# hpcaitech/CachedEmbedding

Measured on AMD Instinct MI355X. Metric: embedding lookups/sec (cache op + EmbeddingBag fwd + bwd/SGD), Criteo-1TB table @1% cache, higher is better.
Workload: dtype f32

## Files before the change

### cachedembedding_amd/csrc/ce_bag.hip

```cpp
#include <stdlib.h>

#include <algorithm>

#include "ce_common.h"

namespace ce {

#ifdef CE_ABLATIONS
#define CE_DBG(x) (x)
#else
#define CE_DBG(x) 0
#endif

struct BagParams {
  const float* weight;
  float* dst;
  const float* grad_out;
  const int64_t* indices;
  const void* offsets;
  const float* psw;
  int64_t nnz;
  int32_t num_bags;
  int32_t rowlen;
  int32_t g_log2;
// ... 303 lines not shown
  return lo;
}

template <typename KT> struct KeyOps;
template <> struct KeyOps<uint32_t> {
  static __device__ __forceinline__ uint32_t make(uint32_t row, int i) { return (row << 10) | (uint32_t)i; }
  static __device__ __forceinline__ uint32_t row(uint32_t k) { return k >> 10; }
  static __device__ __forceinline__ int idx(uint32_t k) { return (int)(k & 1023u); }
  static __device__ __forceinline__ uint32_t invalid() { return 0xffffffffu; }
  static __device__ __forceinline__ uint32_t row_invalid() { return 0x3fffffu; }
};
template <> struct KeyOps<unsigned long long> {
  static __device__ __forceinline__ unsigned long long make(uint32_t row, int i) {
    return ((unsigned long long)row << 32) | (uint32_t)i;
  }
  static __device__ __forceinline__ uint32_t row(unsigned long long k) { return (uint32_t)(k >> 32); }
  static __device__ __forceinline__ int idx(unsigned long long k) { return (int)(uint32_t)k; }
  static __device__ __forceinline__ unsigned long long invalid() { return ~0ull; }
  static __device__ __forceinline__ uint32_t row_invalid() { return 0xffffffffu; }
};

template <typename KT>
__device__ __forceinline__ KT shfl_xor_key(KT v, int m) { return __shfl_xor(v, m); }
template <>
__device__ __forceinline__ unsigned long long shfl_xor_key<unsigned long long>(unsigned long long v, int m) {
  const unsigned lo = __shfl_xor((unsigned)v, m), hi = __shfl_xor((unsigned)(v >> 32), m);
  return ((unsigned long long)hi << 32) | lo;
}

template <typename KT>
__device__ __forceinline__ void tile_sort_1024(KT (&key)[4], KT* lds, int tid) {
  for (int k = 2; k <= kBwdTile; k <<= 1) {
    for (int j = k >> 1; j > 0; j >>= 1) {
      if (j >= 256) {
#pragma unroll
        for (int r = 0; r < 4; ++r) lds[tid * 4 + r] = key[r];
        __syncthreads();
#pragma unroll
        for (int r = 0; r < 4; ++r) {
          const int i = tid * 4 + r;
          const KT other = lds[i ^ j];
          const bool lower = (i & j) == 0, up = (i & k) == 0;
          const KT lo = key[r] < other ? key[r] : other, hi = key[r] < other ? other : key[r];
          key[r] = (lower == up) ? lo : hi;
        }
        __syncthreads();
      } else if (j >= 4) {
#pragma unroll
        for (int r = 0; r < 4; ++r) {
          const int i = tid * 4 + r;
          const KT other = shfl_xor_key<KT>(key[r], j >> 2);
          const bool lower = (i & j) == 0, up = (i & k) == 0;
          const KT lo = key[r] < other ? key[r] : other, hi = key[r] < other ? other : key[r];
          key[r] = (lower == up) ? lo : hi;
        }
      } else {
#pragma unroll
        for (int r = 0; r < 4; ++r) {
          if (r & j) continue;
          const bool up = ((tid * 4 + r) & k) == 0;
          const KT a = key[r], b = key[r | j];
          if ((a > b) == up) {
            key[r] = b;
            key[r | j] = a;
          }
        }
      }
    }
  }
#pragma unroll
  for (int r = 0; r < 4; ++r) lds[tid * 4 + r] = key[r];
  __syncthreads();
}

constexpr int kSegLen = 16384;
constexpr int kSegKeys = 16;
#ifndef CE_SEG_BUCKETS
#define CE_SEG_BUCKETS 8192
#endif
constexpr int kSegBuckets = CE_SEG_BUCKETS;
constexpr int kExclRun = 32;
constexpr unsigned kExclFlag = 0x80000000u;

template <bool SRC, bool EXCL, bool ROWS>
__global__ __launch_bounds__(1024) void k_bag_presort_seg(const int64_t* __restrict__ indices, int64_t nnz_per_batch,
                                                         int32_t segs_per_batch, int64_t n_segs, uint32_t num_rows,
                                                         unsigned long long* __restrict__ keys_out, BagParams lay,
                                                         int64_t off_stride, const int64_t* __restrict__ ids,
                                                         int64_t* __restrict__ ids_minmax, int64_t* slots_io,
                                                         const int32_t* __restrict__ inverted,
                                                         const int* __restrict__ status) {
  __shared__ unsigned long long lk[kSegLen];
  static_assert(sizeof(unsigned long long) * kSegLen <= 160 * 1024 - 1024, "gfx950: 160 KB of LDS per CU");
  int* const cnt = (int*)lk;
  __shared__ int wsum[16];
  __shared__ long long mm_s[2][16];
  const int tid = threadIdx.x, lane = tid & 63, wv = tid >> 6;
  for (int64_t seg = blockIdx.x; seg < n_segs; seg += gridDim.x) {
    const int64_t batch = seg / segs_per_batch;
    const int sib = (int)(seg - batch * segs_per_batch);
    const int64_t in_base = batch * nnz_per_batch + (int64_t)sib * kSegLen;
    const int64_t base = seg * kSegLen;
    const int n_here = (int)min((int64_t)kSegLen, nnz_per_batch - (int64_t)sib * kSegLen);
    BagParams q = lay;
    if (SRC && lay.offsets) q.offsets = (const char*)lay.offsets + batch * off_stride * (lay.off64 ? 8 : 4);
    for (int i = tid; i <= kSegBuckets; i += 1024) cnt[i] = 0;
    __syncthreads();
    unsigned long long key[kSegKeys];
    int place[kSegKeys], bkt[kSegKeys];
    int32_t slot_r[ROWS ? kSegKeys : 1];
    if (ROWS) {
      const bool failed = *status != CE_OK;
      int32_t row_r[kSegKeys];
#pragma unroll
      for (int r = 0; r < kSegKeys; ++r) {
        const int e = r * 1024 + tid;
        row_r[r] = e < n_here ? (int32_t)slots_io[in_base + e] : -1;
      }
#pragma unroll
      for (int r = 0; r < kSegKeys; ++r) slot_r[r] = (row_r[r] >= 0 && !failed) ? inverted[row_r[r]] : -1;
#pragma unroll
      for (int r = 0; r < kSegKeys; ++r) {
        const int e = r * 1024 + tid;
        if (e < n_here) slots_io[in_base + e] = (int64_t)slot_r[r];
      }
    }
#pragma unroll
    for (int r = 0; r < kSegKeys; ++r) {
      const int e = r * 1024 + tid;
      key[r] = ~0ull;
      bkt[r] = kSegBuckets;
      if (e < n_here) {
        const int64_t row = ROWS ? (int64_t)slot_r[ROWS ? r : 0] : indices[in_base + e];
        const bool valid = (uint64_t)row < (uint64_t)num_rows;
        if (valid || SRC) {
          unsigned low = (unsigned)e;
          if (SRC && !(CE_DBG(lay.debug) & 2))
            low = (unsigned)out_row(q, lay.offsets ? find_bag(q, sib * kSegLen + e) : sib * kSegLen + e);
          key[r] = ((unsigned long long)(valid ? (uint32_t)row : 0xffffffffu) << 32) | low;
          if (valid) bkt[r] = (int)(row & (kSegBuckets - 1));
        }
      }
      if (CE_DBG(lay.debug) & 8) {
        place[r] = 0;
        continue;
      }
      const int b0 = __builtin_amdgcn_readfirstlane(bkt[r]);
      if (__all(bkt[r] == b0)) {
        int first = 0;
        if (lane == 0) first = atomicAdd(&cnt[b0], 64);
        place[r] = __shfl(first, 0) + lane;
      } else {
        place[r] = atomicAdd(&cnt[bkt[r]], 1);
      }
    }
    __syncthreads();
    constexpr int kPer = kSegBuckets / 1024;
    int c4[kPer], sum = 0;
#pragma unroll
    for (int q = 0; q < kPer; ++q) { c4[q] = cnt[tid * kPer + q]; sum += c4[q]; }
    int inc = sum;
#pragma unroll
    for (int d = 1; d < 64; d <<= 1) {
      const int o = __shfl_up(inc, d);
      if (lane >= d) inc += o;
    }
    if (lane == 63) wsum[wv] = inc;
    __syncthreads();
    int pre = inc - sum;
    for (int k = 0; k < wv; ++k) pre += wsum[k];
    int total = 0;
    for (int k = 0; k < 16; ++k) total += wsum[k];
#pragma unroll
    for (int q = 0; q < kPer; ++q) { cnt[tid * kPer + q] = pre; pre += c4[q]; }
    if (tid == 0) cnt[kSegBuckets] = total;
    __syncthreads();
    if (!EXCL) {
      int pos[kSegKeys];
#pragma unroll
      for (int r = 0; r < kSegKeys; ++r) pos[r] = cnt[bkt[r]] + place[r];
      __syncthreads();
#pragma unroll
      for (int r = 0; r < kSegKeys; ++r) lk[pos[r]] = key[r];
      __syncthreads();
#pragma unroll
      for (int r = 0; r < kSegKeys; ++r) keys_out[base + r * 1024 + tid] = lk[r * 1024 + tid];
      __syncthreads();
      continue;
    }
    int pos[kSegKeys];
#pragma unroll
    for (int r = 0; r < kSegKeys; ++r) pos[r] = cnt[bkt[r]] + place[r];
    __syncthreads();
#pragma unroll
    for (int r = 0; r < kSegKeys; ++r) lk[pos[r]] = key[r];
    __syncthreads();
    {
      const uint32_t* hi = (const uint32_t*)lk;
      const int p0 = tid * kSegKeys;
      for (int p = p0; p < p0 + kSegKeys; ++p) {
        const uint32_t row = hi[2 * p + 1];
        if (row == 0xffffffffu) break;
        const uint32_t b = row & (kSegBuckets - 1);
        if (p > 0 && (hi[2 * p - 1] & (kSegBuckets - 1)) == b && hi[2 * p - 1] != 0xffffffffu) continue;
        int e = p + 1;
        while (e < kSegLen && e - p <= kExclRun && hi[2 * e + 1] != 0xffffffffu && (hi[2 * e + 1] & (kSegBuckets - 1)) == b) ++e;
        if (e - p > kExclRun) continue;
        for (int i = p + 1; i < e; ++i) {
          const unsigned long long k = lk[i];
          int j = i;
          while (j > p && (uint32_t)(lk[j - 1] >> 32) > (uint32_t)(k >> 32)) { lk[j] = lk[j - 1]; --j; }
          lk[j] = k;
        }
        for (int a = p; a < e;) {
          int z = a + 1;
          while (z < e && (uint32_t)(lk[z] >> 32) == (uint32_t)(lk[a] >> 32)) ++z;
          if ((a >> 4) == ((z - 1) >> 4)) lk[a] |= kExclFlag;
          a = z;
        }
      }
    }
    __syncthreads();
#pragma unroll
    for (int r = 0; r < kSegKeys; ++r) keys_out[base + r * 1024 + tid] = lk[r * 1024 + tid];
    if (ids_minmax) {
      long long lo = INT64_MAX, hi2 = INT64_MIN;
      if (ids) {
#pragma unroll
        for (int r = 0; r < kSegKeys; ++r) {
          const int e = r * 1024 + tid;
          if (e < n_here) {
            const long long v = ids[in_base + e];
            lo = v < lo ? v : lo;
            hi2 = v > hi2 ? v : hi2;
          }
        }
      } else {
        lo = INT64_MIN; hi2 = INT64_MAX;
      }
#pragma unroll
      for (int d = 32; d >= 1; d >>= 1) {
        const long long ol = __shfl_xor(lo, d), oh = __shfl_xor(hi2, d);
        lo = ol < lo ? ol : lo;
        hi2 = oh > hi2 ? oh : hi2;
      }
      if (lane == 0) { mm_s[0][wv] = lo; mm_s[1][wv] = hi2; }
      __syncthreads();
      if (tid == 0) {
        for (int k = 1; k < 16; ++k) {
          lo = mm_s[0][k] < lo ? mm_s[0][k] : lo;
          hi2 = mm_s[1][k] > hi2 ? mm_s[1][k] : hi2;
        }
        ids_minmax[2 * seg] = lo;
        ids_minmax[2 * seg + 1] = hi2;
      }
    }
    __syncthreads();
  }
}

template <typename VT, int NCH, typename KT, int R>
__global__ __launch_bounds__(256) void k_bag_bwd_tile(BagParams p) {
  using K = KeyOps<KT>;
  __shared__ KT keys[kBwdTile];
  __shared__ int bagl[kBwdTile];
  __shared__ float scl[kBwdTile];

  const int tid = threadIdx.x;
  const int G = 1 << p.g_log2;
  const int ngroups = 256 >> p.g_log2;
  const int grp = tid >> p.g_log2;
  const int gl = tid & (G - 1);
  const int rowlen = p.rowlen;
  const int dim = rowlen * (int)(sizeof(VT) / 4);
  const VT* __restrict__ GO = (const VT*)p.grad_out;
  const int tile_len = p.tile_len;
  const int64_t total = p.presorted ? ((p.nnz + kSegLen - 1) / kSegLen) * kSegLen : p.nnz;
  const int ntiles = (int)((total + tile_len - 1) / tile_len);

  for (int tile = blockIdx.x; tile < ntiles; tile += gridDim.x) {
    const int j0 = tile * tile_len;
    const int nv = min(tile_len, (int)(total - j0));
    const bool presorted = p.presorted != nullptr;
    KT kr[4];
#pragma unroll
    for (int r = 0; r < 4; ++r) {
      const int i = tid * 4 + r;
      kr[r] = K::invalid();
      int j = j0 + i;
      uint32_t row = 0xffffffffu;
      if (presorted) {
        const unsigned long long sk = i < nv ? p.presorted[(int64_t)j0 + i] : ~0ull;
        j = -1;
        if (sk != ~0ull) {
          row = (uint32_t)(sk >> 32);
          j = (int)((((int64_t)j0 + i) / kSegLen) * kSegLen) + (int)(uint32_t)sk;
        }
      } else if (i < nv) {
        const int64_t r64 = p.indices[j];
        if ((uint64_t)r64 < (uint64_t)p.num_rows) row = (uint32_t)r64;
      } else {
        j = -1;
      }
      if (j >= 0) {
        const int bag = find_bag(p, j);
        float sc = p.alpha;
        if (p.psw) sc *= p.psw[j];
        if (p.mode == CE_MODE_MEAN) {
          const int len = bag_end(p, bag) - ld_off(p, bag);
          if (len > 1) sc = sc / (float)len;
        }
        bagl[i] = (int)out_row(p, bag);
        scl[i] = sc;
        if (row != 0xffffffffu) kr[r] = K::make(row, i);
      }
    }
    if (CE_DBG(p.debug) == 3) { __syncthreads(); continue; }
    if (presorted) {
#pragma unroll
      for (int r = 0; r < 4; ++r) keys[tid * 4 + r] = kr[r];
      __syncthreads();
    } else {
      tile_sort_1024<KT>(kr, keys, tid);
    }
    if (CE_DBG(p.debug) == 4) continue;
    const int kChunk = (nv + ngroups - 1) / ngroups;
    const int nchunks = (nv + kChunk - 1) / kChunk;
    for (int ck = grp; ck < nchunks; ck += ngroups) {
      const int s0 = ck * kChunk, s1 = min(nv, s0 + kChunk);
      VT acc[NCH];
#pragma unroll
      for (int c = 0; c < NCH; ++c) acc[c] = vzero<VT>();
      uint32_t cur = K::row(keys[s0]);
      for (int q = s0; q < s1; q += R) {
        VT v[R][NCH];
        float sc[R];
        uint32_t rw[R];
#pragma unroll
        for (int t = 0; t < R; ++t) {
          const KT key = (q + t < s1) ? keys[q + t] : K::invalid();
          const bool on = key != K::invalid();
          const int li = on ? K::idx(key) : 0;
          rw[t] = on ? K::row(key) : K::row_invalid();
          sc[t] = on ? scl[li] : 0.f;
          const int64_t orow = bagl[li];
#pragma unroll
          for (int c = 0; c < NCH; ++c) {
            const int ch = gl + c * G;
            v[t][c] = vzero<VT>();
            if (on && ch < rowlen) v[t][c] = __builtin_nontemporal_load(&GO[orow * rowlen + ch]);
          }
        }
        __builtin_amdgcn_s_waitcnt(0x0F70);
#pragma unroll
        for (int t = 0; t < R; ++t) {
          if (rw[t] != K::row_invalid()) {
            if (rw[t] != cur) {
#pragma unroll
              for (int c = 0; c < NCH; ++c) {
                if (cur != K::row_invalid())
                  flush_chunk(p.dst + (int64_t)cur * dim, acc[c], gl, G, c, rowlen, CE_DBG(p.debug));
                acc[c] = vzero<VT>();
              }
              cur = rw[t];
            }
#pragma unroll
            for (int c = 0; c < NCH; ++c) acc[c] = acc[c] + v[t][c] * sc[t];
          }
        }
      }
#pragma unroll
      for (int c = 0; c < NCH; ++c) {
        if (cur != K::row_invalid()) flush_chunk(p.dst + (int64_t)cur * dim, acc[c], gl, G, c, rowlen, CE_DBG(p.debug));
      }
    }
    __syncthreads();
  }
}

template <typename VT, int NCH, int R, bool NTG, bool EXCL>
__global__ __launch_bounds__(256) void k_bag_bwd_stream(BagParams p, int64_t total, const long long* __restrict__ seg_ranges) {
  __shared__ unsigned long long lk[256 * (R > 4 ? R : 4)];
  const int tid = threadIdx.x;
  const int G = 1 << p.g_log2;
  const int ngroups = 256 >> p.g_log2;
  const int grp = tid >> p.g_log2;
  const int gl = tid & (G - 1);
  const int rowlen = p.rowlen;
  const int dim = rowlen * (int)(sizeof(VT) / 4);
  const VT* __restrict__ GO = (const VT*)p.grad_out;
  const VT* __restrict__ WV = (const VT*)p.dst;
  const unsigned long long* __restrict__ keys = p.presorted;
  bool excl = false;
  if (EXCL) {
    const int nseg = (int)(total / kSegLen);
    int clash = nseg > 64 || seg_ranges == nullptr;
    if (!clash) {
      for (int pr = tid; pr < nseg * nseg; pr += 256) {
        const int a = pr / nseg, b2 = pr - a * nseg;
        if (a >= b2) continue;
        const long long alo = seg_ranges[2 * a], ahi = seg_ranges[2 * a + 1];
        const long long blo = seg_ranges[2 * b2], bhi = seg_ranges[2 * b2 + 1];
        if (alo <= ahi && blo <= bhi && !(ahi < blo || bhi < alo)) clash = 1;
      }
    }
    excl = __syncthreads_or(clash) == 0;
  }
  const int64_t all_groups = (int64_t)gridDim.x * ngroups;
  const int64_t round = R > 16 ? R : 16;
  const int64_t share = ((total + all_groups - 1) / all_groups + round - 1) / round * round;
  const int64_t s0 = share_of(p, grp, ngroups) * share;
  const int64_t s1 = min(total, s0 + share);
  if (s0 >= s1) return;
  const float alpha = p.alpha;
  const int kc = 4 * G > R ? 4 * G : R;
  unsigned long long* mylk = lk + grp * kc;
  VT acc[NCH];
#pragma unroll
  for (int c = 0; c < NCH; ++c) acc[c] = vzero<VT>();
  uint32_t cur = 0xffffffffu;
  bool cur_excl = false;
  for (int64_t c0 = s0; c0 < s1; c0 += kc) {
    for (int k = gl; k < kc; k += G) mylk[k] = c0 + k < s1 ? keys[c0 + k] : ~0ull;
    const int64_t c1 = min(s1, c0 + kc);
    for (int64_t q = c0; q < c1; q += R) {
      VT v[R][NCH];
      VT w2[EXCL ? R : 1][NCH];
      uint32_t rw[R];
      uint32_t heads = 0;
#pragma unroll
      for (int t = 0; t < R; ++t) {
        const unsigned long long k = mylk[(int)(q - c0) + t];
        const bool on = k != ~0ull && (uint32_t)(k >> 32) < p.num_rows;
        rw[t] = on ? (uint32_t)(k >> 32) : 0xffffffffu;
        const uint32_t low = (uint32_t)k;
        const int64_t src = (int64_t)(low & ~kExclFlag);
        const bool head = EXCL && excl && on && (low & kExclFlag);
        if (head) heads |= 1u << t;
#pragma unroll
        for (int c = 0; c < NCH; ++c) {
          const int ch = gl + c * G;
          v[t][c] = vzero<VT>();
          if (on && ch < rowlen) v[t][c] = NTG ? __builtin_nontemporal_load(&GO[src * rowlen + ch]) : GO[src * rowlen + ch];
          if (EXCL) {
            w2[t][c] = vzero<VT>();
            if (head && ch < rowlen) w2[t][c] = WV[(int64_t)rw[t] * rowlen + ch];
          }
        }
      }
      __builtin_amdgcn_s_waitcnt(0x0F70);
#pragma unroll
      for (int t = 0; t < R; ++t) {
        if (rw[t] != 0xffffffffu) {
          const bool head = EXCL && ((heads >> t) & 1);
          if (rw[t] != cur || head) {
#pragma unroll
            for (int c = 0; c < NCH; ++c) {
              if (cur != 0xffffffffu) {
                if (EXCL && cur_excl) {
                  const int ch = gl + c * G;
                  if (ch < rowlen) ((VT*)(p.dst + (int64_t)cur * dim))[ch] = acc[c];
                } else {
                  flush_chunk(p.dst + (int64_t)cur * dim, acc[c], gl, G, c, rowlen, CE_DBG(p.debug));
                }
              }
              acc[c] = EXCL ? w2[EXCL ? t : 0][c] : vzero<VT>();
            }
            cur = rw[t];
            cur_excl = head;
          }
#pragma unroll
          for (int c = 0; c < NCH; ++c) acc[c] = acc[c] + v[t][c] * alpha;
        }
      }
    }
  }
  if (cur != 0xffffffffu) {
#pragma unroll
    for (int c = 0; c < NCH; ++c) {
      if (EXCL && cur_excl) {
        const int ch = gl + c * G;
        if (ch < rowlen) ((VT*)(p.dst + (int64_t)cur * dim))[ch] = acc[c];
      } else {
        flush_chunk(p.dst + (int64_t)cur * dim, acc[c], gl, G, c, rowlen, CE_DBG(p.debug));
      }
    }
  }
}

template <typename VT, int NCH, int R, int NTS>
__global__ __launch_bounds__(256, 4) void k_bag_fwd_keys(BagParams p, int64_t total) {
  __shared__ unsigned long long lk[256 * (R > 4 ? R : 4)];
  const int tid = threadIdx.x;
  const int G = 1 << p.g_log2;
  const int ngroups = 256 >> p.g_log2;
  const int grp = tid >> p.g_log2;
  const int gl = tid & (G - 1);
  const int rowlen = p.rowlen;
  const VT* __restrict__ W = (const VT*)p.weight;
  VT* __restrict__ O = (VT*)p.dst;
  const unsigned long long* __restrict__ keys = p.presorted;
  const int64_t all_groups = (int64_t)gridDim.x * ngroups;
  const int64_t round = R > 16 ? R : 16;
  const int64_t share = ((total + all_groups - 1) / all_groups + round - 1) / round * round;
  const int64_t s0 = share_of(p, grp, ngroups) * share;
  const int64_t s1 = min(total, s0 + share);
  if (s0 >= s1) return;
  const int kc = 4 * G > R ? 4 * G : R;
  unsigned long long* mylk = lk + grp * kc;
  VT prev[NCH];
#pragma unroll
  for (int c = 0; c < NCH; ++c) prev[c] = vzero<VT>();
  uint32_t prev_row = 0xffffffffu;
  for (int64_t c0 = s0; c0 < s1; c0 += kc) {
    for (int k = gl; k < kc; k += G) mylk[k] = c0 + k < s1 ? keys[c0 + k] : ~0ull;
    const int64_t c1 = min(s1, c0 + kc);
    for (int64_t q = c0; q < c1; q += R) {
      VT v[R][NCH];
      uint32_t heads = 0;
      uint32_t last = prev_row;
#pragma unroll
      for (int t = 0; t < R; ++t) {
        const unsigned long long k = mylk[(int)(q - c0) + t];
        const bool on = k != ~0ull;
        const uint32_t rw = (uint32_t)(k >> 32);
        const bool head = on && rw != last;
        if (on) last = rw;
        if (head) heads |= 1u << t;
#pragma unroll
        for (int c = 0; c < NCH; ++c) {
          const int ch = gl + c * G;
          v[t][c] = vzero<VT>();
          if (head && ch < rowlen && rw < p.num_rows) v[t][c] = W[(int64_t)rw * rowlen + ch];
        }
      }
      __builtin_amdgcn_s_waitcnt(0x0F70);
#pragma unroll
      for (int t = 0; t < R; ++t) {
        const unsigned long long k = mylk[(int)(q - c0) + t];
        if (k == ~0ull) continue;
        if ((heads >> t) & 1) {
#pragma unroll
          for (int c = 0; c < NCH; ++c) prev[c] = v[t][c];
        }
        const int64_t orow = (int64_t)((uint32_t)k & ~kExclFlag);
#pragma unroll
        for (int c = 0; c < NCH; ++c) {
          const int ch = gl + c * G;
          if (ch < rowlen) store_out<NTS>(&O[orow * rowlen + ch], prev[c]);
        }
      }
      prev_row = last;
    }
  }
}

template <typename VT, int NCH>
__global__ __launch_bounds__(256) void k_rows_axpy(float* __restrict__ dst, uint32_t num_rows,
                                                   const int64_t* __restrict__ index, int64_t n,
                                                   const VT* __restrict__ src, int rowlen, int g_log2, int dim,
                                                   float alpha) {
  constexpr int U = (NCH == 1) ? 8 : (NCH == 2 ? 4 : 2);
  const int lane = threadIdx.x & 63;
  const int G = 1 << g_log2;
  const int gpw = 64 >> g_log2;
  const int grp = lane >> g_log2;
  const int gl = lane & (G - 1);
  const int wpb = blockDim.x >> 6;
  const int64_t wave = (int64_t)blockIdx.x * wpb + (threadIdx.x >> 6);
  const int64_t nwaves = (int64_t)gridDim.x * wpb;
  const int64_t per_wave = (int64_t)gpw * U;
  for (int64_t r0 = wave * per_wave; r0 < n; r0 += nwaves * per_wave) {
    VT v[U][NCH];
    int64_t row[U];
#pragma unroll
// ... 154 lines not shown
                               int32_t include_last_offset, const float* per_sample_weights, int32_t mode,
                               int64_t hook_features, const float* grad_out, const unsigned long long* presorted,
                               ce_stream_t stream) {
  if (num_bags == 0 || nnz == 0) return CE_OK;
  CE_REQUIRE(grad_weight && grad_out && offsets && indices, CE_ERR_INVALID, "null pointer");
  BagParams p{};
  bool vec;
  int nch;
  int rc = fill_params(p, dim, indices, nnz, offsets, offsets_are_i64, num_bags, include_last_offset,
                       per_sample_weights, mode, hook_features, &vec, &nch, grad_weight, grad_out, nullptr);
  if (rc) return rc;
  p.dst = grad_weight;
  p.grad_out = grad_out;
  p.alpha = 1.f;
  CE_REQUIRE(num_rows > 0 && num_rows < (int64_t)INT32_MAX, CE_ERR_INVALID, "num_rows out of range");
  p.num_rows = (uint32_t)num_rows;
  p.presorted = presorted;
  return launch_bwd_scatter(p, vec, nch, (hipStream_t)stream);
}

extern "C" int ce_bag_backward_dense(float* grad_weight, int64_t num_rows, int32_t dim, const int64_t* indices,
                                     int64_t nnz, const void* offsets, int32_t offsets_are_i64,
                                     int64_t num_bags, int32_t include_last_offset,
                                     const float* per_sample_weights, int32_t mode, int64_t hook_features,
                                     const float* grad_out, ce_stream_t stream) {
  return backward_dense_impl(grad_weight, num_rows, dim, indices, nnz, offsets, offsets_are_i64, num_bags,
                             include_last_offset, per_sample_weights, mode, hook_features, grad_out, nullptr, stream);
}

extern "C" int ce_bag_backward_dense_presorted(float* grad_weight, int64_t num_rows, int32_t dim,
                                               const int64_t* indices, int64_t nnz, const void* offsets,
                                               int32_t offsets_are_i64, int64_t num_bags,
                                               int32_t include_last_offset, const float* per_sample_weights,
                                               int32_t mode, int64_t hook_features, const float* grad_out,
                                               const uint64_t* presorted_keys, ce_stream_t stream) {
  CE_REQUIRE(presorted_keys, CE_ERR_INVALID, "null presorted_keys");
  return backward_dense_impl(grad_weight, num_rows, dim, indices, nnz, offsets, offsets_are_i64, num_bags,
                             include_last_offset, per_sample_weights, mode, hook_features, grad_out,
                             (const unsigned long long*)presorted_keys, stream);
}

static int backward_sgd_impl(float* weight, int64_t num_rows, int32_t dim, const int64_t* indices, int64_t nnz,
                             const void* offsets, int32_t offsets_are_i64, int64_t num_bags,
                             int32_t include_last_offset, const float* per_sample_weights, int32_t mode,
                             int64_t hook_features, const float* grad_out, float lr,
                             const unsigned long long* presorted, ce_stream_t stream) {
  if (num_bags == 0 || nnz == 0) return CE_OK;
  CE_REQUIRE(weight && grad_out && offsets && indices, CE_ERR_INVALID, "null pointer");
  BagParams p{};
  bool vec;
  int nch;
  int rc = fill_params(p, dim, indices, nnz, offsets, offsets_are_i64, num_bags, include_last_offset,
                       per_sample_weights, mode, hook_features, &vec, &nch, weight, grad_out, nullptr);
  if (rc) return rc;
  p.dst = weight;
  p.grad_out = grad_out;
  p.alpha = -lr;
  CE_REQUIRE(num_rows > 0 && num_rows < (int64_t)INT32_MAX, CE_ERR_INVALID, "num_rows out of range");
  p.num_rows = (uint32_t)num_rows;
  p.presorted = presorted;
  return launch_bwd_scatter(p, vec, nch, (hipStream_t)stream);
}

extern "C" int ce_bag_backward_sgd(float* weight, int64_t num_rows, int32_t dim, const int64_t* indices,
                                   int64_t nnz, const void* offsets, int32_t offsets_are_i64, int64_t num_bags,
                                   int32_t include_last_offset, const float* per_sample_weights, int32_t mode,
                                   int64_t hook_features, const float* grad_out, float lr, ce_stream_t stream) {
  return backward_sgd_impl(weight, num_rows, dim, indices, nnz, offsets, offsets_are_i64, num_bags,
                           include_last_offset, per_sample_weights, mode, hook_features, grad_out, lr, nullptr, stream);
}

extern "C" int ce_bag_backward_sgd_presorted(float* weight, int64_t num_rows, int32_t dim, const int64_t* indices,
                                             int64_t nnz, const void* offsets, int32_t offsets_are_i64,
                                             int64_t num_bags, int32_t include_last_offset,
                                             const float* per_sample_weights, int32_t mode, int64_t hook_features,
                                             const float* grad_out, float lr, const uint64_t* presorted_keys,
                                             ce_stream_t stream) {
  CE_REQUIRE(presorted_keys, CE_ERR_INVALID, "null presorted_keys");
  return backward_sgd_impl(weight, num_rows, dim, indices, nnz, offsets, offsets_are_i64, num_bags,
                           include_last_offset, per_sample_weights, mode, hook_features, grad_out, lr,
                           (const unsigned long long*)presorted_keys, stream);
}

static int launch_bwd_stream(float* dst, int64_t num_rows, int32_t dim, int64_t nnz, const float* grad_out,
                             float alpha, const unsigned long long* keys, const int64_t* seg_ranges, hipStream_t s) {
  if (nnz == 0) return CE_OK;
  CE_REQUIRE(dst && grad_out && keys, CE_ERR_INVALID, "null pointer");
  CE_REQUIRE(num_rows > 0 && num_rows < (int64_t)INT32_MAX, CE_ERR_INVALID, "num_rows out of range");
  BagParams p{};
  bool vec;
  int nch;
  int rc = fill_params(p, dim, nullptr, nnz, nullptr, 0, 0, 1, nullptr, CE_MODE_SUM, 0, &vec, &nch, dst, grad_out,
                       nullptr);
  if (rc) return rc;
  p.dst = dst;
  p.grad_out = grad_out;
  p.alpha = alpha;
  p.num_rows = (uint32_t)num_rows;
  p.presorted = keys;
#ifdef CE_ABLATIONS
  { const char* dbg = getenv("CE_BWD_DEBUG"); p.debug = dbg ? atoi(dbg) : 0; }
#endif
  p.interleave = 1;
  const int64_t total = cdiv(nnz, kSegLen) * kSegLen;
  constexpr int per_cu = 6;
  const int ngroups = 256 >> p.g_log2;
  const int grid = (int)std::max<int64_t>(1, std::min<int64_t>((int64_t)kNumCU * per_cu, cdiv(total, (int64_t)ngroups * 16)));
  dim3 g(grid), b(256);
  const long long* rg = (const long long*)seg_ranges;
  const bool excl = seg_ranges != nullptr && vec && nch == 1;
  if (vec) {
    if (nch == 1 && excl) hipLaunchKernelGGL((k_bag_bwd_stream<f32x4, 1, 16, true, true>), g, b, 0, s, p, total, rg);
    else if (nch == 1) hipLaunchKernelGGL((k_bag_bwd_stream<f32x4, 1, 16, true, false>), g, b, 0, s, p, total, rg);
    else if (nch == 2) hipLaunchKernelGGL((k_bag_bwd_stream<f32x4, 2, 8, true, false>), g, b, 0, s, p, total, rg);
    else hipLaunchKernelGGL((k_bag_bwd_stream<f32x4, 4, 4, true, false>), g, b, 0, s, p, total, rg);
  } else {
    if (nch == 1) hipLaunchKernelGGL((k_bag_bwd_stream<float, 1, 16, true, false>), g, b, 0, s, p, total, rg);
    else if (nch == 2) hipLaunchKernelGGL((k_bag_bwd_stream<float, 2, 8, true, false>), g, b, 0, s, p, total, rg);
    else hipLaunchKernelGGL((k_bag_bwd_stream<float, 4, 4, true, false>), g, b, 0, s, p, total, rg);
  }
  CE_LAUNCH_CHECK();
  return CE_OK;
}

extern "C" int ce_bag_backward_sgd_presorted_src(float* weight, int64_t num_rows, int32_t dim, int64_t nnz,
                                                 const float* grad_out, float lr, const uint64_t* src_keys,
                                                 ce_stream_t stream) {
  return launch_bwd_stream(weight, num_rows, dim, nnz, grad_out, -lr, (const unsigned long long*)src_keys, nullptr,
                           (hipStream_t)stream);
}

extern "C" int ce_bag_backward_sgd_presorted_src_excl(float* weight, int64_t num_rows, int32_t dim, int64_t nnz,
                                                      const float* grad_out, float lr, const uint64_t* src_keys,
                                                      const int64_t* seg_id_ranges, ce_stream_t stream) {
  return launch_bwd_stream(weight, num_rows, dim, nnz, grad_out, -lr, (const unsigned long long*)src_keys,
                           seg_id_ranges, (hipStream_t)stream);
}

extern "C" int ce_bag_backward_dense_presorted_src(float* grad_weight, int64_t num_rows, int32_t dim, int64_t nnz,
                                                   const float* grad_out, const uint64_t* src_keys,
                                                   ce_stream_t stream) {
  return launch_bwd_stream(grad_weight, num_rows, dim, nnz, grad_out, 1.f, (const unsigned long long*)src_keys, nullptr,
                           (hipStream_t)stream);
}

extern "C" int ce_bag_forward_src_keys(const float* weight, int64_t num_rows, int32_t dim, int64_t nnz,
                                       const uint64_t* src_keys, float* out, ce_stream_t stream) {
  if (nnz == 0) return CE_OK;
  CE_REQUIRE(weight && src_keys && out, CE_ERR_INVALID, "null pointer");
  CE_REQUIRE(num_rows > 0 && num_rows < (int64_t)INT32_MAX, CE_ERR_INVALID, "num_rows out of range");
  BagParams p{};
  bool vec;
  int nch;
  int rc = fill_params(p, dim, nullptr, nnz, nullptr, 0, 0, 1, nullptr, CE_MODE_SUM, 0, &vec, &nch, weight, out, nullptr);
  if (rc) return rc;
  p.weight = weight;
  p.dst = out;
  p.num_rows = (uint32_t)num_rows;
  p.presorted = (const unsigned long long*)src_keys;
  p.interleave = 0;
  const int64_t total = cdiv(nnz, kSegLen) * kSegLen;
  constexpr int per_cu = 16;
  const int ngroups = 256 >> p.g_log2;
  const int grid = (int)std::max<int64_t>(1, std::min<int64_t>((int64_t)kNumCU * per_cu, cdiv(total, (int64_t)ngroups * 16)));
  dim3 g(grid), b(256);
  hipStream_t s = (hipStream_t)stream;
#define CE_FWK(VT, N, R) hipLaunchKernelGGL((k_bag_fwd_keys<VT, N, R, 1>), g, b, 0, s, p, total)
  if (vec) {
    if (nch == 1) CE_FWK(f32x4, 1, 16);
    else if (nch == 2) CE_FWK(f32x4, 2, 8); else CE_FWK(f32x4, 4, 4);
  } else {
    if (nch == 1) CE_FWK(float, 1, 16); else if (nch == 2) CE_FWK(float, 2, 8); else CE_FWK(float, 4, 4);
  }
#undef CE_FWK
  CE_LAUNCH_CHECK();
  return CE_OK;
}

extern "C" int64_t ce_bag_presort_len(int64_t nnz) { return nnz <= 0 ? 0 : cdiv(nnz, kSegLen) * kSegLen; }

static int presort_window_impl(const int64_t* indices, int64_t nnz_per_batch, int64_t n_batches, int64_t num_rows,
                               uint64_t* keys_out, const BagParams* lay, int64_t off_stride, const int64_t* ids,
                               int64_t* ids_minmax, ce_stream_t stream) {
  if (nnz_per_batch == 0 || n_batches == 0) return CE_OK;
  CE_REQUIRE(indices && keys_out && nnz_per_batch > 0 && n_batches > 0, CE_ERR_INVALID, "bad arguments");
  CE_REQUIRE(nnz_per_batch < (int64_t)INT32_MAX - kSegLen, CE_ERR_INVALID, "batch too large");
  CE_REQUIRE(num_rows > 0 && num_rows < (int64_t)INT32_MAX, CE_ERR_INVALID, "num_rows out of range");
  const int64_t spb = cdiv(nnz_per_batch, kSegLen);
  const int64_t nseg = spb * n_batches;
  CE_REQUIRE(spb < (int64_t)INT32_MAX && nseg < (int64_t)INT32_MAX, CE_ERR_INVALID, "too many segments");
  const dim3 grid((unsigned)std::min<int64_t>(nseg, kMaxBlocks)), block(1024);
  int64_t* const no_io = nullptr;
  const int32_t* const no_inv = nullptr;
  const int* const no_st = nullptr;
  if (lay && ids_minmax)
    hipLaunchKernelGGL((k_bag_presort_seg<true, true, false>), grid, block, 0, (hipStream_t)stream, indices, nnz_per_batch,
                       (int32_t)spb, nseg, (uint32_t)num_rows, (unsigned long long*)keys_out, *lay, off_stride, ids,
                       ids_minmax, no_io, no_inv, no_st);
  else if (lay)
    hipLaunchKernelGGL((k_bag_presort_seg<true, false, false>), grid, block, 0, (hipStream_t)stream, indices, nnz_per_batch,
                       (int32_t)spb, nseg, (uint32_t)num_rows, (unsigned long long*)keys_out, *lay, off_stride,
                       (const int64_t*)nullptr, (int64_t*)nullptr, no_io, no_inv, no_st);
  else
    hipLaunchKernelGGL((k_bag_presort_seg<false, false, false>), grid, block, 0, (hipStream_t)stream, indices, nnz_per_batch,
                       (int32_t)spb, nseg, (uint32_t)num_rows, (unsigned long long*)keys_out, BagParams{}, 0ll,
                       (const int64_t*)nullptr, (int64_t*)nullptr, no_io, no_inv, no_st);
  CE_LAUNCH_CHECK();
  return CE_OK;
}

namespace ce {
int presort_window_from_rows(int64_t* slots_io, int64_t nnz_per_batch, int64_t n_batches, int64_t num_rows,
                             const int32_t* inverted, const int* status, int32_t src_keys, const void* offsets,
                             int32_t offsets_are_i64, int64_t offsets_batch_stride, int64_t num_bags,
                             int32_t include_last_offset, int64_t hook_features, uint64_t* keys_out, hipStream_t stream) {
  if (nnz_per_batch == 0 || n_batches == 0) return CE_OK;
  CE_REQUIRE(slots_io && keys_out && inverted && status && nnz_per_batch > 0 && n_batches > 0, CE_ERR_INVALID, "bad arguments");
  CE_REQUIRE(nnz_per_batch < (int64_t)INT32_MAX - kSegLen, CE_ERR_INVALID, "batch too large");
  CE_REQUIRE(num_rows > 0 && num_rows < (int64_t)INT32_MAX, CE_ERR_INVALID, "num_rows out of range");
  const int64_t spb = cdiv(nnz_per_batch, kSegLen);
  const int64_t nseg = spb * n_batches;
  CE_REQUIRE(spb < (int64_t)INT32_MAX && nseg < (int64_t)INT32_MAX, CE_ERR_INVALID, "too many segments");
  const dim3 grid((unsigned)std::min<int64_t>(nseg, kMaxBlocks)), block(1024);
  if (src_keys) {
    CE_REQUIRE(num_bags > 0 && offsets_batch_stride >= 0, CE_ERR_INVALID, "bad offsets");
    CE_REQUIRE(offsets || num_bags == nnz_per_batch, CE_ERR_INVALID,
               "offsets may only be NULL for the one-id-per-bag layout (num_bags == nnz_per_batch)");
    BagParams lay{};
    bool vec;
    int nch;
    int rc = fill_params(lay, 4, nullptr, nnz_per_batch, offsets, offsets_are_i64, num_bags, include_last_offset, nullptr,
                         CE_MODE_SUM, hook_features, &vec, &nch, nullptr, nullptr, nullptr);
    if (rc) return rc;
    hipLaunchKernelGGL((k_bag_presort_seg<true, false, true>), grid, block, 0, stream, (const int64_t*)nullptr,
                       nnz_per_batch, (int32_t)spb, nseg, (uint32_t)num_rows, (unsigned long long*)keys_out, lay,
                       offsets_batch_stride, (const int64_t*)nullptr, (int64_t*)nullptr, slots_io, inverted, status);
  } else {
    hipLaunchKernelGGL((k_bag_presort_seg<false, false, true>), grid, block, 0, stream, (const int64_t*)nullptr,
                       nnz_per_batch, (int32_t)spb, nseg, (uint32_t)num_rows, (unsigned long long*)keys_out, BagParams{},
                       0ll, (const int64_t*)nullptr, (int64_t*)nullptr, slots_io, inverted, status);
  }
  CE_LAUNCH_CHECK();
  return CE_OK;
}
}

extern "C" int ce_bag_presort_window(const int64_t* indices, int64_t nnz_per_batch, int64_t n_batches,
                                     int64_t num_rows, uint64_t* keys_out, ce_stream_t stream) {
  return presort_window_impl(indices, nnz_per_batch, n_batches, num_rows, keys_out, nullptr, 0, nullptr, nullptr, stream);
}

static int presort_window_src_impl(const int64_t* indices, int64_t nnz_per_batch, int64_t n_batches, int64_t num_rows,
                                   const void* offsets, int32_t offsets_are_i64, int64_t offsets_batch_stride,
                                   int64_t num_bags, int32_t include_last_offset, int64_t hook_features,
                                   const int64_t* ids, uint64_t* keys_out, int64_t* seg_id_ranges, ce_stream_t stream) {
  if (nnz_per_batch == 0 || n_batches == 0) return CE_OK;
  CE_REQUIRE(num_bags > 0 && offsets_batch_stride >= 0, CE_ERR_INVALID, "bad offsets");
  CE_REQUIRE(offsets || num_bags == nnz_per_batch, CE_ERR_INVALID,
             "offsets may only be NULL for the one-id-per-bag layout (num_bags == nnz_per_batch)");
  BagParams lay{};
  bool vec;
  int nch;
  int rc = fill_params(lay, 4, indices, nnz_per_batch, offsets, offsets_are_i64, num_bags, include_last_offset,
                       nullptr, CE_MODE_SUM, hook_features, &vec, &nch, nullptr, nullptr, nullptr);
  if (rc) return rc;
#ifdef CE_ABLATIONS
  { const char* dbg = getenv("CE_PRESORT_DEBUG"); lay.debug = dbg ? atoi(dbg) : 0; }
#endif
  return presort_window_impl(indices, nnz_per_batch, n_batches, num_rows, keys_out, &lay, offsets_batch_stride, ids,
                             seg_id_ranges, stream);
}

extern "C" int ce_bag_presort_window_src(const int64_t* indices, int64_t nnz_per_batch, int64_t n_batches,
                                         int64_t num_rows, const void* offsets, int32_t offsets_are_i64,
                                         int64_t offsets_batch_stride, int64_t num_bags, int32_t include_last_offset,
                                         int64_t hook_features, uint64_t* keys_out, ce_stream_t stream) {
  return presort_window_src_impl(indices, nnz_per_batch, n_batches, num_rows, offsets, offsets_are_i64,
                                 offsets_batch_stride, num_bags, include_last_offset, hook_features, nullptr, keys_out,
                                 nullptr, stream);
}

extern "C" int ce_bag_presort_window_src_excl(const int64_t* indices, int64_t nnz_per_batch, int64_t n_batches,
                                              int64_t num_rows, const void* offsets, int32_t offsets_are_i64,
                                              int64_t offsets_batch_stride, int64_t num_bags,
                                              int32_t include_last_offset, int64_t hook_features, const int64_t* ids,
                                              uint64_t* keys_out, int64_t* seg_id_ranges, ce_stream_t stream) {
  CE_REQUIRE(seg_id_ranges, CE_ERR_INVALID, "null seg_id_ranges");
  return presort_window_src_impl(indices, nnz_per_batch, n_batches, num_rows, offsets, offsets_are_i64,
                                 offsets_batch_stride, num_bags, include_last_offset, hook_features, ids, keys_out,
                                 seg_id_ranges, stream);
}

extern "C" int ce_bag_presort(const int64_t* indices, int64_t nnz, int64_t num_rows, uint64_t* keys_out,
                              ce_stream_t stream) {
  return ce_bag_presort_window(indices, nnz, 1, num_rows, keys_out, stream);
}

extern "C" int ce_rows_axpy(float* weight, int64_t num_rows, int32_t dim, const int64_t* index, int64_t n,
                            const float* src_rows, float alpha, ce_stream_t stream) {
  if (n == 0) return CE_OK;
  CE_REQUIRE(weight && index && src_rows, CE_ERR_INVALID, "null pointer");
  CE_REQUIRE(dim > 0 && n > 0 && n < (int64_t)INT32_MAX, CE_ERR_INVALID, "bad sizes");
  CE_REQUIRE(num_rows > 0 && num_rows < (int64_t)INT32_MAX, CE_ERR_INVALID, "num_rows out of range");
  auto al16 = [](const void* q) { return (((uintptr_t)q) & 15) == 0; };
  const bool vec = (dim % 4 == 0) && al16(weight) && al16(src_rows);
  const int rowlen = vec ? dim / 4 : dim;
// ... 41 lines not shown
```

Measured before the change: 3.305 billion.

## Shrink presort LDS and registers so it co-resides with training kernels

Reworks the segmented presort kernel to use half-size LDS staging for the non-exclusive path, written in two passes. It keeps 32-bit rows plus packed 16-bit places in registers instead of 64-bit keys, and launches one block per segment instead of a grid-stride loop. Launch bounds request more waves per CU. Forward and backward key kernels switch to dynamically sized LDS based on group size, cutting their shared-memory footprint. The goal is to let the side-stream presort overlap with training steps, at the cost of recomputing bag lookups per pass and more complex code. A probe script measuring co-residency is added.

```diff
diff --git a/cachedembedding_amd/csrc/ce_bag.hip b/cachedembedding_amd/csrc/ce_bag.hip
--- a/cachedembedding_amd/csrc/ce_bag.hip
+++ b/cachedembedding_amd/csrc/ce_bag.hip
@@ -409,79 +409,121 @@
 constexpr int kExclRun = 32;
 constexpr unsigned kExclFlag = 0x80000000u;
 
+__device__ __forceinline__ void exclusive_runs(unsigned long long* lk, int tid) {
+  const uint32_t* hi = (const uint32_t*)lk;
+  const int p0 = tid * kSegKeys;
+  for (int p = p0; p < p0 + kSegKeys; ++p) {
+    const uint32_t row = hi[2 * p + 1];
+    if (row == 0xffffffffu) break;
+    const uint32_t b = row & (kSegBuckets - 1);
+    if (p > 0 && (hi[2 * p - 1] & (kSegBuckets - 1)) == b && hi[2 * p - 1] != 0xffffffffu) continue;
+    int e = p + 1;
+    while (e < kSegLen && e - p <= kExclRun && hi[2 * e + 1] != 0xffffffffu && (hi[2 * e + 1] & (kSegBuckets - 1)) == b) ++e;
+    if (e - p > kExclRun) continue;
+    for (int i = p + 1; i < e; ++i) {
+      const unsigned long long k = lk[i];
+      int j = i;
+      while (j > p && (uint32_t)(lk[j - 1] >> 32) > (uint32_t)(k >> 32)) { lk[j] = lk[j - 1]; --j; }
+      lk[j] = k;
+    }
+    for (int a = p; a < e;) {
+      int z = a + 1;
+      while (z < e && (uint32_t)(lk[z] >> 32) == (uint32_t)(lk[a] >> 32)) ++z;
+      if ((a >> 4) == ((z - 1) >> 4)) lk[a] |= kExclFlag;
+      a = z;
+    }
+  }
+}
+
 template <bool SRC, bool EXCL, bool ROWS>
-__global__ __launch_bounds__(1024) void k_bag_presort_seg(const int64_t* __restrict__ indices, int64_t nnz_per_batch,
-                                                         int32_t segs_per_batch, int64_t n_segs, uint32_t num_rows,
-                                                         unsigned long long* __restrict__ keys_out, BagParams lay,
-                                                         int64_t off_stride, const int64_t* __restrict__ ids,
-                                                         int64_t* __restrict__ ids_minmax, int64_t* slots_io,
-                                                         const int32_t* __restrict__ inverted,
-                                                         const int* __restrict__ status) {
-  __shared__ unsigned long long lk[kSegLen];
-  static_assert(sizeof(unsigned long long) * kSegLen <= 160 * 1024 - 1024, "gfx950: 160 KB of LDS per CU");
+__global__ __launch_bounds__(1024, EXCL ? 4 : 8) void k_bag_presort_seg(const int64_t* __restrict__ indices,
+                                                                       int64_t nnz_per_batch, int32_t segs_per_batch,
+                                                                       int64_t n_segs, uint32_t num_rows,
+                                                                       unsigned long long* __restrict__ keys_out,
+                                                                       BagParams lay, int64_t off_stride,
+                                                                       const int64_t* __restrict__ ids,
+                                                                       int64_t* __restrict__ ids_minmax,
+                                                                       int64_t* slots_io,
+                                                                       const int32_t* __restrict__ inverted,
+                                                                       const int* __restrict__ status) {
+  constexpr int kStage = EXCL ? kSegLen : kSegLen / 2;
+  __shared__ unsigned long long lk[kStage];
+  static_assert(sizeof(unsigned long long) * kStage <= 160 * 1024 - 1024, "gfx950: 160 KB of LDS per CU");
+  static_assert(sizeof(int) * (kSegBuckets + 1) <= sizeof(lk), "the bucket counters share the key buffer");
+  static_assert(kSegLen <= 0x10000, "places and positions are 16-bit fields");
   int* const cnt = (int*)lk;
   __shared__ int wsum[16];
   __shared__ long long mm_s[2][16];
-  const int tid = threadIdx.x, lane = tid & 63, wv = tid >> 6;
-  for (int64_t seg = blockIdx.x; seg < n_segs; seg += gridDim.x) {
-    const int64_t batch = seg / segs_per_batch;
-    const int sib = (int)(seg - batch * segs_per_batch);
-    const int64_t in_base = batch * nnz_per_batch + (int64_t)sib * kSegLen;
-    const int64_t base = seg * kSegLen;
+  const int seg = blockIdx.x;
+  if (seg >= n_segs) return;
+  {
+    int tid = threadIdx.x;
+    asm volatile("" : "+v"(tid));
+    const int batch = seg / segs_per_batch;
+    const int sib = seg - batch * segs_per_batch;
+    const int64_t in_base = (int64_t)batch * nnz_per_batch + (int64_t)sib * kSegLen;
+    const int64_t base = (int64_t)seg * kSegLen;
     const int n_here = (int)min((int64_t)kSegLen, nnz_per_batch - (int64_t)sib * kSegLen);
     BagParams q = lay;
     if (SRC && lay.offsets) q.offsets = (const char*)lay.offsets + batch * off_stride * (lay.off64 ? 8 : 4);
     for (int i = tid; i <= kSegBuckets; i += 1024) cnt[i] = 0;
     __syncthreads();
-    unsigned long long key[kSegKeys];
-    int place[kSegKeys], bkt[kSegKeys];
-    int32_t slot_r[ROWS ? kSegKeys : 1];
+    uint32_t rw[kSegKeys];
+    uint32_t pp[kSegKeys / 2];
     if (ROWS) {
       const bool failed = *status != CE_OK;
-      int32_t row_r[kSegKeys];
+      const int32_t* const rows32 = (const int32_t*)(slots_io + in_base);
 #pragma unroll
       for (int r = 0; r < kSegKeys; ++r) {
         const int e = r * 1024 + tid;
-        row_r[r] = e < n_here ? (int32_t)slots_io[in_base + e] : -1;
-      }
-#pragma unroll
-      for (int r = 0; r < kSegKeys; ++r) slot_r[r] = (row_r[r] >= 0 && !failed) ? inverted[row_r[r]] : -1;
+        const int32_t row = rows32[2 * min(e, n_here - 1)];
+        rw[r] = (e < n_here && row >= 0 && !failed) ? (uint32_t)row : 0xffffffffu;
+      }
+#pragma unroll
+      for (int r = 0; r < kSegKeys; ++r) {
+        const int32_t slot = inverted[rw[r] == 0xffffffffu ? 0 : rw[r]];
+        rw[r] = rw[r] == 0xffffffffu ? 0xffffffffu : (uint32_t)slot;
+      }
+      asm volatile("" : "+v"(tid));
 #pragma unroll
       for (int r = 0; r < kSegKeys; ++r) {
         const int e = r * 1024 + tid;
-        if (e < n_here) slots_io[in_base + e] = (int64_t)slot_r[r];
-      }
-    }
+        if (e < n_here) slots_io[in_base + e] = (int64_t)(int32_t)rw[r];
+        if (rw[r] >= num_rows) rw[r] = 0xffffffffu;
+      }
+    } else {
+#pragma unroll
+      for (int r = 0; r < kSegKeys; ++r) {
+        const int e = r * 1024 + tid;
+        const int64_t row = indices[in_base + min(e, n_here - 1)];
+        rw[r] = (e < n_here && (uint64_t)row < (uint64_t)num_rows) ? (uint32_t)row : 0xffffffffu;
+      }
+    }
+    asm volatile("" : "+v"(tid));
+    auto bucket = [](uint32_t row) { return row == 0xffffffffu ? kSegBuckets : (int)(row & (kSegBuckets - 1)); };
 #pragma unroll
     for (int r = 0; r < kSegKeys; ++r) {
-      const int e = r * 1024 + tid;
-      key[r] = ~0ull;
-      bkt[r] = kSegBuckets;
-      if (e < n_here) {
-        const int64_t row = ROWS ? (int64_t)slot_r[ROWS ? r : 0] : indices[in_base + e];
-        const bool valid = (uint64_t)row < (uint64_t)num_rows;
-        if (valid || SRC) {
-          unsigned low = (unsigned)e;
-          if (SRC && !(CE_DBG(lay.debug) & 2))
-            low = (unsigned)out_row(q, lay.offsets ? find_bag(q, sib * kSegLen + e) : sib * kSegLen + e);
-          key[r] = ((unsigned long long)(valid ? (uint32_t)row : 0xffffffffu) << 32) | low;
-          if (valid) bkt[r] = (int)(row & (kSegBuckets - 1));
-        }
-      }
-      if (CE_DBG(lay.debug) & 8) {
-        place[r] = 0;
-        continue;
-      }
-      const int b0 = __builtin_amdgcn_readfirstlane(bkt[r]);
-      if (__all(bkt[r] == b0)) {
-        int first = 0;
-        if (lane == 0) first = atomicAdd(&cnt[b0], 64);
-        place[r] = __shfl(first, 0) + lane;
-      } else {
-        place[r] = atomicAdd(&cnt[bkt[r]], 1);
-      }
-    }
+      const int b = bucket(rw[r]);
+      int place = 0;
+      if (!(CE_DBG(lay.debug) & 8)) {
+        const int b0 = __builtin_amdgcn_readfirstlane(b);
+        if (__all(b == b0)) {
+          int first = 0;
+          if ((tid & 63) == 0) first = atomicAdd(&cnt[b0], 64);
+          place = __builtin_amdgcn_readfirstlane(first) + (tid & 63);
+        } else {
+          place = atomicAdd(&cnt[b], 1);
+        }
+      }
+      pp[r >> 1] = (r & 1) ? pp[r >> 1] | (uint32_t)place << 16 : (uint32_t)place;
+    }
+#pragma unroll
+    for (int r = 0; r < kSegKeys; ++r) asm volatile("" : "+v"(rw[r]));
+#pragma unroll
+    for (int i = 0; i < kSegKeys / 2; ++i) asm volatile("" : "+v"(pp[i]));
     __syncthreads();
+    asm volatile("" : "+v"(tid));
+    const int lane = tid & 63, wv = tid >> 6;
     constexpr int kPer = kSegBuckets / 1024;
     int c4[kPer], sum = 0;
 #pragma unroll
@@ -494,62 +536,51 @@
     }
     if (lane == 63) wsum[wv] = inc;
     __syncthreads();
-    int pre = inc - sum;
-    for (int k = 0; k < wv; ++k) pre += wsum[k];
-    int total = 0;
-    for (int k = 0; k < 16; ++k) total += wsum[k];
+    int pre = inc - sum, total = 0;
+#pragma unroll
+    for (int k = 0; k < 16; ++k) {
+      const int w = wsum[k];
+      total += w;
+      pre += k < wv ? w : 0;
+    }
 #pragma unroll
     for (int q = 0; q < kPer; ++q) { cnt[tid * kPer + q] = pre; pre += c4[q]; }
     if (tid == 0) cnt[kSegBuckets] = total;
     __syncthreads();
-    if (!EXCL) {
-      int pos[kSegKeys];
-#pragma unroll
-      for (int r = 0; r < kSegKeys; ++r) pos[r] = cnt[bkt[r]] + place[r];
+#pragma unroll
+    for (int i = 0; i < kSegKeys / 2; ++i) {
+      const uint32_t p0 = (uint32_t)cnt[bucket(rw[2 * i])] + (pp[i] & 0xffffu);
+      const uint32_t p1 = (uint32_t)cnt[bucket(rw[2 * i + 1])] + (pp[i] >> 16);
+      pp[i] = p0 | p1 << 16;
+    }
+    __syncthreads();
+    for (int h = 0; h < kSegLen / kStage; ++h) {
+      asm volatile("" : "+v"(tid));
+      if (SRC) asm volatile("" : "+s"(q.hookB));
+#pragma unroll
+      for (int r = 0; r < kSegKeys; ++r) {
+        const int e = r * 1024 + tid;
+        const int pos = (int)((pp[r >> 1] >> (16 * (r & 1))) & 0xffffu) - h * kStage;
+        if (pos < 0 || pos >= kStage) continue;
+        uint32_t low = (unsigned)e;
+        if (SRC && e < n_here && !(CE_DBG(lay.debug) & 2))
+          low = (unsigned)out_row(q, lay.offsets ? find_bag(q, sib * kSegLen + e) : sib * kSegLen + e);
+        uint32_t row;
+        asm volatile("v_mov_b32 %0, %1" : "=v"(row) : "v"(rw[r]));
+        unsigned long long key = ~0ull;
+        if (e < n_here && (SRC || row != 0xffffffffu)) key = (unsigned long long)row << 32 | low;
+        lk[pos] = key;
+      }
       __syncthreads();
-#pragma unroll
-      for (int r = 0; r < kSegKeys; ++r) lk[pos[r]] = key[r];
+      if (EXCL) {
+        exclusive_runs(lk, tid);
+        __syncthreads();
+      }
+#pragma unroll
+      for (int r = 0; r < kStage / 1024; ++r) keys_out[base + h * kStage + r * 1024 + tid] = lk[r * 1024 + tid];
       __syncthreads();
-#pragma unroll
-      for (int r = 0; r < kSegKeys; ++r) keys_out[base + r * 1024 + tid] = lk[r * 1024 + tid];
-      __syncthreads();
-      continue;
-    }
-    int pos[kSegKeys];
-#pragma unroll
-    for (int r = 0; r < kSegKeys; ++r) pos[r] = cnt[bkt[r]] + place[r];
-    __syncthreads();
-#pragma unroll
-    for (int r = 0; r < kSegKeys; ++r) lk[pos[r]] = key[r];
-    __syncthreads();
-    {
-      const uint32_t* hi = (const uint32_t*)lk;
-      const int p0 = tid * kSegKeys;
-      for (int p = p0; p < p0 + kSegKeys; ++p) {
-        const uint32_t row = hi[2 * p + 1];
-        if (row == 0xffffffffu) break;
-        const uint32_t b = row & (kSegBuckets - 1);
-        if (p > 0 && (hi[2 * p - 1] & (kSegBuckets - 1)) == b && hi[2 * p - 1] != 0xffffffffu) continue;
-        int e = p + 1;
-        while (e < kSegLen && e - p <= kExclRun && hi[2 * e + 1] != 0xffffffffu && (hi[2 * e + 1] & (kSegBuckets - 1)) == b) ++e;
-        if (e - p > kExclRun) continue;
-        for (int i = p + 1; i < e; ++i) {
-          const unsigned long long k = lk[i];
-          int j = i;
-          while (j > p && (uint32_t)(lk[j - 1] >> 32) > (uint32_t)(k >> 32)) { lk[j] = lk[j - 1]; --j; }
-          lk[j] = k;
-        }
-        for (int a = p; a < e;) {
-          int z = a + 1;
-          while (z < e && (uint32_t)(lk[z] >> 32) == (uint32_t)(lk[a] >> 32)) ++z;
-          if ((a >> 4) == ((z - 1) >> 4)) lk[a] |= kExclFlag;
-          a = z;
-        }
-      }
-    }
-    __syncthreads();
-#pragma unroll
-    for (int r = 0; r < kSegKeys; ++r) keys_out[base + r * 1024 + tid] = lk[r * 1024 + tid];
+    }
+    if (!EXCL) return;
     if (ids_minmax) {
       long long lo = INT64_MAX, hi2 = INT64_MIN;
       if (ids) {
@@ -582,7 +613,6 @@
         ids_minmax[2 * seg + 1] = hi2;
       }
     }
-    __syncthreads();
   }
 }
 
@@ -707,7 +737,7 @@
 
 template <typename VT, int NCH, int R, bool NTG, bool EXCL>
 __global__ __launch_bounds__(256) void k_bag_bwd_stream(BagParams p, int64_t total, const long long* __restrict__ seg_ranges) {
-  __shared__ unsigned long long lk[256 * (R > 4 ? R : 4)];
+  extern __shared__ __attribute__((aligned(16))) unsigned long long lk[];
   const int tid = threadIdx.x;
   const int G = 1 << p.g_log2;
   const int ngroups = 256 >> p.g_log2;
@@ -817,7 +847,7 @@
 
 template <typename VT, int NCH, int R, int NTS>
 __global__ __launch_bounds__(256, 4) void k_bag_fwd_keys(BagParams p, int64_t total) {
-  __shared__ unsigned long long lk[256 * (R > 4 ? R : 4)];
+  extern __shared__ __attribute__((aligned(16))) unsigned long long lk[];
   const int tid = threadIdx.x;
   const int G = 1 << p.g_log2;
   const int ngroups = 256 >> p.g_log2;
@@ -1138,6 +1168,11 @@
                            (const unsigned long long*)presorted_keys, stream);
 }
 
+static size_t key_slice_bytes(const BagParams& p, int R) {
+  const int G = 1 << p.g_log2;
+  return (size_t)(256 >> p.g_log2) * (size_t)std::max(4 * G, R) * sizeof(unsigned long long);
+}
+
 static int launch_bwd_stream(float* dst, int64_t num_rows, int32_t dim, int64_t nnz, const float* grad_out,
                              float alpha, const unsigned long long* keys, const int64_t* seg_ranges, hipStream_t s) {
   if (nnz == 0) return CE_OK;
@@ -1165,15 +1200,16 @@
   dim3 g(grid), b(256);
   const long long* rg = (const long long*)seg_ranges;
   const bool excl = seg_ranges != nullptr && vec && nch == 1;
+  const size_t lds = key_slice_bytes(p, nch == 1 ? 16 : nch == 2 ? 8 : 4);
   if (vec) {
-    if (nch == 1 && excl) hipLaunchKernelGGL((k_bag_bwd_stream<f32x4, 1, 16, true, true>), g, b, 0, s, p, total, rg);
-    else if (nch == 1) hipLaunchKernelGGL((k_bag_bwd_stream<f32x4, 1, 16, true, false>), g, b, 0, s, p, total, rg);
-    else if (nch == 2) hipLaunchKernelGGL((k_bag_bwd_stream<f32x4, 2, 8, true, false>), g, b, 0, s, p, total, rg);
-    else hipLaunchKernelGGL((k_bag_bwd_stream<f32x4, 4, 4, true, false>), g, b, 0, s, p, total, rg);
+    if (nch == 1 && excl) hipLaunchKernelGGL((k_bag_bwd_stream<f32x4, 1, 16, true, true>), g, b, lds, s, p, total, rg);
+    else if (nch == 1) hipLaunchKernelGGL((k_bag_bwd_stream<f32x4, 1, 16, true, false>), g, b, lds, s, p, total, rg);
+    else if (nch == 2) hipLaunchKernelGGL((k_bag_bwd_stream<f32x4, 2, 8, true, false>), g, b, lds, s, p, total, rg);
+    else hipLaunchKernelGGL((k_bag_bwd_stream<f32x4, 4, 4, true, false>), g, b, lds, s, p, total, rg);
   } else {
-    if (nch == 1) hipLaunchKernelGGL((k_bag_bwd_stream<float, 1, 16, true, false>), g, b, 0, s, p, total, rg);
-    else if (nch == 2) hipLaunchKernelGGL((k_bag_bwd_stream<float, 2, 8, true, false>), g, b, 0, s, p, total, rg);
-    else hipLaunchKernelGGL((k_bag_bwd_stream<float, 4, 4, true, false>), g, b, 0, s, p, total, rg);
+    if (nch == 1) hipLaunchKernelGGL((k_bag_bwd_stream<float, 1, 16, true, false>), g, b, lds, s, p, total, rg);
+    else if (nch == 2) hipLaunchKernelGGL((k_bag_bwd_stream<float, 2, 8, true, false>), g, b, lds, s, p, total, rg);
+    else hipLaunchKernelGGL((k_bag_bwd_stream<float, 4, 4, true, false>), g, b, lds, s, p, total, rg);
   }
   CE_LAUNCH_CHECK();
   return CE_OK;
@@ -1221,7 +1257,7 @@
   const int grid = (int)std::max<int64_t>(1, std::min<int64_t>((int64_t)kNumCU * per_cu, cdiv(total, (int64_t)ngroups * 16)));
   dim3 g(grid), b(256);
   hipStream_t s = (hipStream_t)stream;
-#define CE_FWK(VT, N, R) hipLaunchKernelGGL((k_bag_fwd_keys<VT, N, R, 1>), g, b, 0, s, p, total)
+#define CE_FWK(VT, N, R) hipLaunchKernelGGL((k_bag_fwd_keys<VT, N, R, 1>), g, b, key_slice_bytes(p, R), s, p, total)
   if (vec) {
     if (nch == 1) CE_FWK(f32x4, 1, 16);
     else if (nch == 2) CE_FWK(f32x4, 2, 8); else CE_FWK(f32x4, 4, 4);
@@ -1245,7 +1281,7 @@
   const int64_t spb = cdiv(nnz_per_batch, kSegLen);
   const int64_t nseg = spb * n_batches;
   CE_REQUIRE(spb < (int64_t)INT32_MAX && nseg < (int64_t)INT32_MAX, CE_ERR_INVALID, "too many segments");
-  const dim3 grid((unsigned)std::min<int64_t>(nseg, kMaxBlocks)), block(1024);
+  const dim3 grid((unsigned)nseg), block(1024);
   int64_t* const no_io = nullptr;
   const int32_t* const no_inv = nullptr;
   const int* const no_st = nullptr;
@@ -1277,7 +1313,7 @@
   const int64_t spb = cdiv(nnz_per_batch, kSegLen);
   const int64_t nseg = spb * n_batches;
   CE_REQUIRE(spb < (int64_t)INT32_MAX && nseg < (int64_t)INT32_MAX, CE_ERR_INVALID, "too many segments");
-  const dim3 grid((unsigned)std::min<int64_t>(nseg, kMaxBlocks)), block(1024);
+  const dim3 grid((unsigned)nseg), block(1024);
   if (src_keys) {
     CE_REQUIRE(num_bags > 0 && offsets_batch_stride >= 0, CE_ERR_INVALID, "bad offsets");
     CE_REQUIRE(offsets || num_bags == nnz_per_batch, CE_ERR_INVALID,
diff --git a/profiles/probes/presort_coresidency.py b/profiles/probes/presort_coresidency.py
--- /dev/null
+++ b/profiles/probes/presort_coresidency.py
@@ -0,0 +1,72 @@
+import argparse
+import json
+import statistics
+import sys
+from pathlib import Path
+
+import torch
+
+sys.path.insert(0, str(Path(__file__).resolve().parents[2]))
+from cachedembedding_amd._lib import LIB_PATH, check, lib, ptr
+from cachedembedding_amd.functional import presort_window
+
+
+def main():
+    ap = argparse.ArgumentParser()
+    ap.add_argument("--reps", type=int, default=30)
+    ap.add_argument("--C", type=int, default=1_779_442)
+    ap.add_argument("--distinct", type=float, default=0.105)
+    a = ap.parse_args()
+    B, F, D, P = 16384, 26, 128, 8
+    n = B * F
+    dev = torch.device("cuda")
+    g = torch.Generator(device=dev).manual_seed(7)
+    W = torch.randn(a.C, D, device=dev, generator=g)
+    u = torch.rand(P, n, device=dev, generator=g)
+    slots = (u ** 4 * int(a.distinct * n * 4)).long() % a.C
+    off = torch.arange(n + 1, dtype=torch.int32, device=dev)
+    lay = dict(offsets=off, include_last_offset=True, hook_features=F, identity_bags=True)
+    keys = [k.keys for k in presort_window(slots, a.C, **lay)]
+    win_keys = torch.empty(P, keys[0].numel(), dtype=torch.int64, device=dev)
+    out = torch.empty(n, D, device=dev)
+    go = torch.randn(n, D, device=dev, generator=g) * 1e-3
+    s_train, s_side = torch.cuda.Stream(), torch.cuda.Stream()
+
+    def steps():
+        sp = s_train.cuda_stream
+        for b in range(P):
+            check(lib.ce_bag_forward_src_keys(ptr(W), a.C, D, n, ptr(keys[b]), ptr(out), sp))
+            check(lib.ce_bag_backward_sgd_presorted_src(ptr(W), a.C, D, n, ptr(go), 0.0, ptr(keys[b]), sp))
+
+    def presort():
+        with torch.cuda.stream(s_side):
+            presort_window(slots, a.C, keys_out=win_keys, **lay)
+
+    ev = lambda: torch.cuda.Event(enable_timing=True)
+    res = {"steps_alone": [], "steps_beside_presort": [], "presort_alone": [], "presort_beside_steps": []}
+    for rep in range(a.reps + 3):
+        torch.cuda.synchronize()
+        t0, t1 = ev(), ev()
+        t0.record(s_train); steps(); t1.record(s_train)
+        torch.cuda.synchronize()
+        p0, p1 = ev(), ev()
+        p0.record(s_side); presort(); p1.record(s_side)
+        torch.cuda.synchronize()
+        q0, q1, r0, r1 = ev(), ev(), ev(), ev()
+        q0.record(s_side); presort(); q1.record(s_side)
+        r0.record(s_train); steps(); r1.record(s_train)
+        torch.cuda.synchronize()
+        if rep >= 3:
+            res["steps_alone"].append(t0.elapsed_time(t1))
+            res["presort_alone"].append(p0.elapsed_time(p1))
+            res["presort_beside_steps"].append(q0.elapsed_time(q1))
+            res["steps_beside_presort"].append(r0.elapsed_time(r1))
+    med = {k: round(statistics.median(v), 4) for k, v in res.items()}
+    spread = {k: [round(min(v), 4), round(max(v), 4)] for k, v in res.items()}
+    print(json.dumps({"probe": "presort_coresidency", "library": str(LIB_PATH), "unit": "ms", "reps": a.reps,
+                      "shape": dict(B=B, F=F, D=D, P=P, C=a.C), "median": med, "min_max": spread,
+                      "steps_cost_of_presort_ms": round(med["steps_beside_presort"] - med["steps_alone"], 4)}))
+
+
+if __name__ == "__main__":
+    main()
```

Result: no change. 3.270 billion (median of 2 runs) (-1.1%).
